# abhi1kumar/SUP-NeRF

Hardware: AMD Instinct MI355X
Metric: rays/sec at 4096 rays x 64 samples (fused render forward) (higher is better)
Workload: dtype f32

## Files before the change

sup-nerf_amd/csrc/snr_aux.hip:

```cpp
#include "snr_device.hpp"
#include "snr_host.hpp"

namespace snr {

__global__ void pack_fwd_kernel(const float* __restrict__ Wt, int n_out, int k_in, int n_chunks, float* __restrict__ dst) {
    const long long total = (long long)n_chunks * n_out * KC;
    for (long long i = blockIdx.x * (long long)blockDim.x + threadIdx.x; i < total; i += (long long)gridDim.x * blockDim.x) {
        const int kk = (int)(i % KC);
        const int row = (int)((i / KC) % n_out);
        const int c = (int)(i / ((long long)KC * n_out));
        const int k = c * KC + kk;
        dst[(long long)c * n_out * KC + chunk_pos(row, kk)] = (k < k_in) ? Wt[(long long)row * k_in + k] : 0.f;
    }
}

__global__ void pack_bwd_kernel(const float* __restrict__ Wt, int n_out, int k_in, int rows_pad, float* __restrict__ dst) {
    const int n_chunks = n_out / KC;
    const long long total = (long long)n_chunks * rows_pad * KC;
    for (long long i = blockIdx.x * (long long)blockDim.x + threadIdx.x; i < total; i += (long long)gridDim.x * blockDim.x) {
        const int kk = (int)(i % KC);
        const int row = (int)((i / KC) % rows_pad);
        const int c = (int)(i / ((long long)KC * rows_pad));
        const int n = c * KC + kk;
        dst[(long long)c * rows_pad * KC + chunk_pos(row, kk)] = (row < k_in) ? Wt[(long long)n * k_in + row] : 0.f;
    }
}

__global__ void copy_pad_kernel(const float* __restrict__ src, int n, float* __restrict__ dst, int n_pad) {
    const int i = blockIdx.x * blockDim.x + threadIdx.x;
    if (i < n_pad) dst[i] = (i < n) ? src[i] : 0.f;
}

__global__ void __launch_bounds__(256) composite_fwd_kernel(const float* __restrict__ sigmas, const float* __restrict__ rgbs,
                                                            const float* __restrict__ zv, int z_mode, int flags, long long n_rays,
                                                            long long rays_per_obj, int S, float* __restrict__ rgb,
                                                            float* __restrict__ depth, float* __restrict__ acc) {
    const int lane = threadIdx.x & 63;
    const long long wave0 = (blockIdx.x * (long long)blockDim.x + threadIdx.x) >> 6;
    const long long n_waves = ((long long)gridDim.x * blockDim.x) >> 6;
    const bool white = flags & SNR_WHITE_BKGD;
    for (long long ray = wave0; ray < n_rays; ray += n_waves) {
        const float* zrow = zv + (z_mode == SNR_Z_SHARED ? 0 : (z_mode == SNR_Z_PER_OBJECT ? (ray / rays_per_obj) * S : ray * S));
        const float* srow = sigmas + ray * S;
        const float* crow = rgbs + ray * S * 3;
        RayOut o = composite_ray_fwd(S, lane, white, [&](int k, float& sg, float& cr, float& cg, float& cb, float& z, float& zn) {
            sg = srow[k]; cr = crow[3 * k]; cg = crow[3 * k + 1]; cb = crow[3 * k + 2];
            z = zrow[k]; zn = (k < S - 1) ? zrow[k + 1] : 0.f;
        });
        if (lane == 0) {
            rgb[ray * 3] = o.r; rgb[ray * 3 + 1] = o.g; rgb[ray * 3 + 2] = o.b;
            depth[ray] = o.depth; acc[ray] = o.acc;
        }
    }
}

__global__ void __launch_bounds__(256) composite_fwd16_kernel(const float* __restrict__ sigmas, const float* __restrict__ rgbs,
                                                              const float* __restrict__ zv, int z_mode, int flags, long long n_rays,
                                                              long long rays_per_obj, int S, float* __restrict__ rgb,
                                                              float* __restrict__ depth, float* __restrict__ acc) {
    const int lane = threadIdx.x & 63, sub = lane & 15, grp = lane >> 4;
    const long long wave0 = (blockIdx.x * (long long)blockDim.x + threadIdx.x) >> 6;
    const long long n_waves = ((long long)gridDim.x * blockDim.x) >> 6;
    const bool white = flags & SNR_WHITE_BKGD;
    const int k0 = 4 * sub;
    const bool valid = k0 < S;
    for (long long base = wave0 * 4; base < n_rays; base += n_waves * 4) {
        const long long ray = base + grp;
        const bool live = ray < n_rays && valid;
        const long long rr = ray < n_rays ? ray : n_rays - 1;
        const float* zrow = zv + (z_mode == SNR_Z_SHARED ? 0 : (z_mode == SNR_Z_PER_OBJECT ? (rr / rays_per_obj) * S : rr * S));
        f32x4 sg = {0.f, 0.f, 0.f, 0.f}, z4 = sg, c0 = sg, c1 = sg, c2 = sg;
        if (live) {
            sg = *reinterpret_cast<const f32x4*>(sigmas + rr * S + k0);
            z4 = *reinterpret_cast<const f32x4*>(zrow + k0);
            const f32x4* cp = reinterpret_cast<const f32x4*>(rgbs + (rr * S + k0) * 3);
            c0 = cp[0]; c1 = cp[1]; c2 = cp[2];
        }
        const float zn = dpp_or<0x101>(0.f, z4[0]);
        const float zz[5] = {z4[0], z4[1], z4[2], z4[3], zn};
        const float cr[4] = {c0[0], c0[3], c1[2], c2[1]}, cg[4] = {c0[1], c1[0], c1[3], c2[2]}, cb[4] = {c0[2], c1[1], c2[0], c2[3]};
        float alpha[4], Al[4];
        float prod = 1.f;
#pragma unroll
        for (int e = 0; e < 4; ++e) {
            const int k = k0 + e;
            const float delta = (k == S - 1) ? LAST_DELTA : zz[e + 1] - zz[e];
            alpha[e] = 1.f - expf(-fmaxf(sg[e], 0.f) * delta);
            Al[e] = prod;
            prod *= live ? (1.f - alpha[e]) + TRANS_EPS : 1.f;
        }
        float incl = prod;
        incl *= dpp_or<0x111>(1.f, incl); incl *= dpp_or<0x112>(1.f, incl); incl *= dpp_or<0x114>(1.f, incl); incl *= dpp_or<0x118>(1.f, incl);
        const float excl = dpp_or<0x111>(1.f, incl);
        float sr = 0.f, sgc = 0.f, sb = 0.f, sd = 0.f, sw = 0.f, al = 0.f;
#pragma unroll
        for (int e = 0; e < 4; ++e) {
            const float A = excl * Al[e];
            const float w = live ? alpha[e] * A : 0.f;
            sr += w * cr[e]; sgc += w * cg[e]; sb += w * cb[e]; sd += w * zz[e]; sw += w;
            if (live && k0 + e == S - 1) al = A;
        }
        sr = row_sum(sr); sgc = row_sum(sgc); sb = row_sum(sb); sd = row_sum(sd); sw = row_sum(sw); al = row_sum(al);
        if (white) { const float bg = 1.f - sw; sr += bg; sgc += bg; sb += bg; }
        if (sub == 0 && ray < n_rays) {
            rgb[ray * 3] = sr; rgb[ray * 3 + 1] = sgc; rgb[ray * 3 + 2] = sb;
            depth[ray] = sd; acc[ray] = al;
        }
// ... 383 lines not shown
        v = (f < 3 + 3 * DIR_FREQ) ? sn : cs;
    }
    pe_dir[i] = v;
}

constexpr int RED_CHUNK = 32;
__global__ void __launch_bounds__(256) reduce_tiles_kernel(const float* __restrict__ in, long long tiles, int cols, float* __restrict__ out) {
    const long long n_chunks = (tiles + RED_CHUNK - 1) / RED_CHUNK;
    const long long chunk = blockIdx.x, obj = blockIdx.y;
    const long long t0 = chunk * RED_CHUNK;
    const long long t1 = (t0 + RED_CHUNK < tiles) ? t0 + RED_CHUNK : tiles;
    for (int c4 = threadIdx.x; c4 * 4 < cols; c4 += blockDim.x) {
        const float* p = in + (obj * tiles + t0) * cols + c4 * 4;
        f32x4 s0 = {0.f, 0.f, 0.f, 0.f}, s1 = s0;
        long long t = t0;
        for (; t + 1 < t1; t += 2) {
            s0 += *reinterpret_cast<const f32x4*>(p);
            s1 += *reinterpret_cast<const f32x4*>(p + cols);
            p += 2 * (long long)cols;
        }
        if (t < t1) s0 += *reinterpret_cast<const f32x4*>(p);
        *reinterpret_cast<f32x4*>(out + (obj * n_chunks + chunk) * cols + c4 * 4) = s0 + s1;
    }
}

}

using namespace snr;

int snr_bf16_pack_(const float* const* W, int sb, int tb, float* packed, void* stream_);

static thread_local const char* g_last_err = "";
int snr_check_launch_(void) {
    hipError_t e = hipGetLastError();
    if (e != hipSuccess) { g_last_err = hipGetErrorString(e); return SNR_E_LAUNCH; }
    return SNR_OK;
}

extern "C" {

int snr_abi_version(void) { return SNR_ABI_VERSION; }

const char* snr_last_hip_error(void) { return g_last_err; }

size_t snr_packed_bytes(int sb, int tb) {
    if (sb < 0 || tb < 0 || sb > MAX_BLOCKS || tb > MAX_BLOCKS) return 0;
    return (size_t)make_layout(sb, tb).total * sizeof(float);
}

size_t snr_mask_bytes(int64_t n_points, int sb, int tb) { return (size_t)mask_bytes(n_points, sb, tb); }

static inline int grid_for(long long total, int block = 256, int cap = 4096) {
    long long g = (total + block - 1) / block;
    return (int)(g < 1 ? 1 : (g > cap ? cap : g));
}

int snr_pack_weights(const float* const* t, int n_tensors, int sb, int tb, float* packed, void* stream_) {
    if (!t || !packed || sb < 0 || tb < 0 || sb > MAX_BLOCKS || tb > MAX_BLOCKS) return SNR_E_ARG;
    if (n_tensors != 2 * (sb + tb + 6)) return SNR_E_SHAPE;
    for (int i = 0; i < n_tensors; ++i) if (!t[i]) return SNR_E_ARG;
    hipStream_t st = (hipStream_t)stream_;
    const Layout L = make_layout(sb, tb);
    int ti = 0;
    auto Wp = [&](int i) { return t[2 * i]; };
    auto Bp = [&](int i) { return t[2 * i + 1]; };
    const int i_xyz = ti++;
    int i_shape[MAX_BLOCKS]; for (int j = 0; j < sb; ++j) i_shape[j] = ti++;
    const int i_encshape = ti++;
    const int i_sigma = ti++;
    const int i_view = ti++;
    int i_tex[MAX_BLOCKS]; for (int j = 0; j < tb; ++j) i_tex[j] = ti++;
    const int i_rgb0 = ti++;
    const int i_rgb2 = ti++;
    const long long c256 = 256 * KC;

    float* f = packed + L.fwd;
    auto fwd = [&](const float* Wsrc, int n_out, int k_in, int n_chunks) {
        pack_fwd_kernel<<<grid_for((long long)n_chunks * n_out * KC), 256, 0, st>>>(Wsrc, n_out, k_in, n_chunks, f);
        f += (long long)n_chunks * n_out * KC;
    };
    fwd(Wp(i_xyz), 256, D_XYZ, 2);
    for (int j = 0; j < sb; ++j) fwd(Wp(i_shape[j]), 256, 256, 8);
    fwd(Wp(i_encshape), 256, 256, 8);
    fwd(Wp(i_view), 256, 256 + D_DIR, 9);
    for (int j = 0; j < tb; ++j) fwd(Wp(i_tex[j]), 256, 256, 8);
    fwd(Wp(i_rgb0), 128, 256, 8);
    if (f - (packed + L.fwd) != L.fwd_floats) return SNR_E_SHAPE;

    float* b = packed + L.bwd;
    auto bwd = [&](const float* Wsrc, int n_out, int k_in, int rows_pad) {
        const int n_chunks = n_out / KC;
        pack_bwd_kernel<<<grid_for((long long)n_chunks * rows_pad * KC), 256, 0, st>>>(Wsrc, n_out, k_in, rows_pad, b);
        b += (long long)n_chunks * rows_pad * KC;
    };
    bwd(Wp(i_rgb0), 128, 256, 256);
    for (int j = tb - 1; j >= 0; --j) bwd(Wp(i_tex[j]), 256, 256, 256);
    bwd(Wp(i_view), 256, 256 + D_DIR, K_VIEW_PAD);
    bwd(Wp(i_encshape), 256, 256, 256);
    for (int j = sb - 1; j >= 0; --j) bwd(Wp(i_shape[j]), 256, 256, 256);
    bwd(Wp(i_xyz), 256, D_XYZ, K_XYZ_PAD);
    if (b - (packed + L.bwd) != L.bwd_floats) return SNR_E_SHAPE;
    (void)c256;

    auto vec = [&](const float* src, int n, long long off, int n_pad) {
        copy_pad_kernel<<<(n_pad + 255) / 256, 256, 0, st>>>(src, n, packed + off, n_pad);
    };
    vec(Bp(i_xyz), 256, L.bias + 256ll * layer_enc_xyz(), 256);
    for (int j = 0; j < sb; ++j) vec(Bp(i_shape[j]), 256, L.bias + 256ll * layer_shape(j), 256);
    vec(Bp(i_encshape), 256, L.bias + 256ll * layer_enc_shape(sb), 256);
    vec(Bp(i_view), 256, L.bias + 256ll * layer_viewdir(sb), 256);
    for (int j = 0; j < tb; ++j) vec(Bp(i_tex[j]), 256, L.bias + 256ll * layer_texture(sb, j), 256);
    vec(Bp(i_rgb0), 128, L.bias + 256ll * layer_rgb0(sb, tb), 256);
    vec(Wp(i_sigma), 256, L.sigma_w, 256);
    vec(Bp(i_sigma), 1, L.sigma_b, 4);
    vec(Wp(i_rgb2), 3 * 128, L.rgb2_w, 3 * 128);
    vec(Bp(i_rgb2), 3, L.rgb2_b, 4);
    {
        const float* Wl[MAX_BLOCKS * 2 + 4];
        int n = 0;
        Wl[n++] = Wp(i_xyz);
        for (int j = 0; j < sb; ++j) Wl[n++] = Wp(i_shape[j]);
        Wl[n++] = Wp(i_encshape);
        Wl[n++] = Wp(i_view);
        for (int j = 0; j < tb; ++j) Wl[n++] = Wp(i_tex[j]);
        Wl[n++] = Wp(i_rgb0);
        int rc = snr_bf16_pack_(Wl, sb, tb, packed, stream_);
        if (rc != SNR_OK) return rc;
    }
    return snr_check_launch_();
}

int snr_composite_fwd(const float* sigmas, const float* rgbs, const float* z_vals, int z_mode, int flags, int64_t n_rays,
                      int64_t rays_per_obj, int S, float* rgb, float* depth, float* acc, void* stream_) {
    if (n_rays == 0) return SNR_OK;
    if (!sigmas || !rgbs || !z_vals || !rgb || !depth || !acc) return SNR_E_ARG;
    if (n_rays < 0 || S < 1 || z_mode < 0 || z_mode > 2) return SNR_E_ARG;
    if (z_mode == SNR_Z_PER_OBJECT && (rays_per_obj < 1)) return SNR_E_SHAPE;
    if (rays_per_obj < 1) rays_per_obj = n_rays;
    const bool aligned = !(((uintptr_t)sigmas | (uintptr_t)rgbs | (uintptr_t)z_vals) & 15);
    if (S <= 64 && (S & 3) == 0 && aligned) {
        const int grid = grid_for(n_rays * 16, 256, 16384);
        composite_fwd16_kernel<<<grid, 256, 0, (hipStream_t)stream_>>>(sigmas, rgbs, z_vals, z_mode, flags, n_rays, rays_per_obj, S, rgb, depth, acc);
        return snr_check_launch_();
    }
    const int grid = grid_for(n_rays * 64, 256, 8192);
    composite_fwd_kernel<<<grid, 256, 0, (hipStream_t)stream_>>>(sigmas, rgbs, z_vals, z_mode, flags, n_rays, rays_per_obj, S, rgb, depth, acc);
    return snr_check_launch_();
}

int snr_scene_composite_fwd(const float* sigmas, const float* rgbs, const float* z_vals, int64_t n_pixels, int n_per_pixel, int run_length,
                            int flags, float* rgb, float* depth, float* acc, void* stream_) {
    if (n_pixels == 0) return SNR_OK;
    if (!sigmas || !rgbs || !z_vals || !rgb) return SNR_E_ARG;
    if (n_pixels < 0 || n_per_pixel < 1 || run_length < 0) return SNR_E_ARG;
    if (run_length > 0 && (n_per_pixel % run_length) != 0) return SNR_E_SHAPE;
    const size_t lds = (size_t)4 * 6 * n_per_pixel * sizeof(float);
    if (lds > 160 * 1024) return SNR_E_UNSUPPORTED;
    if (lds > 64 * 1024) {
        hipError_t e = hipFuncSetAttribute(reinterpret_cast<const void*>(scene_general_kernel<false>), hipFuncAttributeMaxDynamicSharedMemorySize, (int)lds);
        if (e != hipSuccess) return snr_check_launch_();
    }
    const int grid = grid_for(n_pixels * 64, 256, 8192);
    hipStream_t st = (hipStream_t)stream_;
    const bool fast = n_per_pixel <= 256 && (run_length == 32 || run_length == 64 || run_length == 128);
    if (fast) {
        if (run_length == 32) scene_fast_kernel<32><<<grid, 256, lds, st>>>(sigmas, rgbs, z_vals, n_pixels, n_per_pixel, flags, rgb, depth, acc);
        else if (run_length == 64) scene_fast_kernel<64><<<grid, 256, lds, st>>>(sigmas, rgbs, z_vals, n_pixels, n_per_pixel, flags, rgb, depth, acc);
        else scene_fast_kernel<128><<<grid, 256, lds, st>>>(sigmas, rgbs, z_vals, n_pixels, n_per_pixel, flags, rgb, depth, acc);
        scene_general_kernel<true><<<grid, 256, lds, st>>>(sigmas, rgbs, z_vals, n_pixels, n_per_pixel, run_length, flags, rgb, depth, acc);
    } else {
        scene_general_kernel<false><<<grid, 256, lds, st>>>(sigmas, rgbs, z_vals, n_pixels, n_per_pixel, run_length, flags, rgb, depth, acc);
    }
    return snr_check_launch_();
}

int snr_composite_bwd(const float* sigmas, const float* rgbs, const float* z_vals, int z_mode, int flags, int64_t n_rays,
                      int64_t rays_per_obj, int S, const float* d_rgb, const float* d_depth, const float* d_acc,
                      float* d_sigmas, float* d_rgbs, float* d_z, void* stream_) {
    if (n_rays == 0) return SNR_OK;
    if (!sigmas || !rgbs || !z_vals || !d_sigmas || !d_rgbs) return SNR_E_ARG;
    if (n_rays < 0 || S < 1 || z_mode < 0 || z_mode > 2) return SNR_E_ARG;
    if (d_z && z_mode != SNR_Z_PER_RAY) return SNR_E_UNSUPPORTED;
    if (S > 256) return SNR_E_UNSUPPORTED;
    if (rays_per_obj < 1) rays_per_obj = n_rays;
    const int grid = grid_for(n_rays * 64, 256, 8192);
    hipStream_t st = (hipStream_t)stream_;
#define SNR_LAUNCH_CB(N) composite_bwd_kernel<N><<<grid, 256, 0, st>>>(sigmas, rgbs, z_vals, z_mode, flags, n_rays, rays_per_obj, S, \
                                                                        d_rgb, d_depth, d_acc, d_sigmas, d_rgbs, d_z)
    if (S <= 64) SNR_LAUNCH_CB(1); else if (S <= 128) SNR_LAUNCH_CB(2); else if (S <= 192) SNR_LAUNCH_CB(3); else SNR_LAUNCH_CB(4);
#undef SNR_LAUNCH_CB
    return snr_check_launch_();
}

int snr_pe_points(const float* xyz, const float* viewdir, int64_t n_points, float* out, void* stream_) {
    if (n_points == 0) return SNR_OK;
    if (!xyz || !viewdir || !out || n_points < 0 || (((uintptr_t)out) & 15)) return SNR_E_ARG;
    pe_points_kernel<<<(unsigned)((n_points + 127) / 128), 256, 0, (hipStream_t)stream_>>>(xyz, viewdir, n_points, out);
    return snr_check_launch_();
}
// ... 63 lines not shown
```

sup-nerf_amd/csrc/snr_layout.h:

```cpp
#pragma once
#include <stdint.h>

#ifndef SNR_HD
#ifdef __HIPCC__
#define SNR_HD __host__ __device__
#else
#define SNR_HD
#endif
#endif

namespace snr {

constexpr int W = 256;
constexpr int W_RGB = 128;
constexpr int XYZ_FREQ = 10;
constexpr int DIR_FREQ = 4;
constexpr int D_XYZ = 3 + 6 * XYZ_FREQ;
constexpr int D_DIR = 3 + 6 * DIR_FREQ;
constexpr int KC = 32;
constexpr int K_XYZ_PAD = 64;
constexpr int K_VIEW_PAD = 288;
constexpr int MAX_BLOCKS = 8;

struct Layout {
    int sb, tb;
    int n_mfma_layers;
    int n_lat;
    int64_t fwd;
    int64_t bwd;
    int64_t bias;
    int64_t sigma_w;
    int64_t sigma_b;
    int64_t rgb2_w;
    int64_t rgb2_b;
    int64_t bf_fwd;
    int64_t bf_bwd;
    int64_t total;
    int64_t fwd_floats, bwd_floats;
    int64_t bf_fwd_bytes, bf_bwd_bytes;
};

constexpr int BF_CHUNK = 32768;
constexpr int BF_CHUNK_VIEW = 36864;

SNR_HD inline Layout make_layout(int sb, int tb) {
    Layout L;
    L.sb = sb; L.tb = tb;
    L.n_mfma_layers = sb + tb + 4;
    L.n_lat = sb + tb;
    const int64_t c256 = 256 * KC;
    L.fwd_floats = 2 * c256 + (int64_t)(sb + 1) * 8 * c256 + 9 * c256 + (int64_t)tb * 8 * c256 + 8 * (128 * KC);
    L.bwd_floats = 4 * c256 + (int64_t)tb * 8 * c256 + 8 * (288 * KC) + (int64_t)(sb + 1) * 8 * c256 + 8 * (64 * KC);
    int64_t o = 0;
    L.fwd = o; o += L.fwd_floats;
    L.bwd = o; o += L.bwd_floats;
    L.bias = o; o += (int64_t)L.n_mfma_layers * 256;
    L.sigma_w = o; o += 256;
    L.sigma_b = o; o += 4;
    L.rgb2_w = o; o += 3 * 128;
    L.rgb2_b = o; o += 4;
    L.bf_fwd_bytes = 2ll * BF_CHUNK + (int64_t)(sb + 1 + tb) * 8 * BF_CHUNK + 8ll * BF_CHUNK_VIEW + 4ll * BF_CHUNK;
    L.bf_bwd_bytes = 4ll * BF_CHUNK + (int64_t)tb * 8 * BF_CHUNK + 9ll * BF_CHUNK + (int64_t)(sb + 1) * 8 * BF_CHUNK + 2ll * BF_CHUNK;
    o = (o + 3) & ~3ll;
    L.bf_fwd = o; o += L.bf_fwd_bytes / 4;
    L.bf_bwd = o; o += L.bf_bwd_bytes / 4;
    L.total = o;
    return L;
}

SNR_HD inline int chunk_pos(int row, int kk) { return row * KC + ((((kk >> 2) ^ ((row >> 1) & 7)) << 2) | (kk & 3)); }

SNR_HD inline int layer_enc_xyz() { return 0; }
SNR_HD inline int layer_shape(int j ) { return 1 + j; }
SNR_HD inline int layer_enc_shape(int sb) { return 1 + sb; }
SNR_HD inline int layer_viewdir(int sb) { return 2 + sb; }
SNR_HD inline int layer_texture(int sb, int j) { return 3 + sb + j; }
SNR_HD inline int layer_rgb0(int sb, int tb) { return 3 + sb + tb; }

SNR_HD inline int n_relu_layers(int sb, int tb) { return sb + tb + 3; }
SNR_HD inline int64_t mask_bytes(int64_t n_points, int sb, int tb) {
    int64_t tiles = (n_points + 31) / 32;
    return tiles * n_relu_layers(sb, tb) * 64 * 16;
}

}
```

sup-nerf_amd/csrc/snr_mlp.hip:

```cpp
#include "snr_mlp_core.hpp"
#include "snr_host.hpp"

namespace snr {

#ifdef SNR_STAMPS
#define SNR32_STAMP(i) do { if (threadIdx.x == 0 && io.sigmas) { unsigned long long t_; asm volatile("s_memtime %0\n\ts_waitcnt lgkmcnt(0)" : "=s"(t_) :: "memory"); \
        reinterpret_cast<unsigned long long*>(io.sigmas)[(long long)blockIdx.x * 16 + 4 + (i)] = t_; } } while (0)
#else
#define SNR32_STAMP(i) do {} while (0)
#endif

__device__ __forceinline__ void decoder_forward_tile(const DecoderIO& io, const Layout& L, float* lds, long long gp , long long tile32,
                                                     float x, float y, float z, float dx, float dy, float dz,
                                                     float& o_sigma, float& o_r, float& o_g, float& o_b) {
    const int tid = threadIdx.x;
    const int lane = tid & 63, wave = tid >> 6;
    const int p = lane & 31, h = lane >> 5;
    const int sb = io.sb, tb = io.tb;
    const int n_relu = n_relu_layers(sb, tb);
    const bool tile_live = tile32 * 32 < io.n_points;
    const int dump_rows = (int)((io.n_points - tile32 * 32) < 32 ? (io.n_points - tile32 * 32) : 32);
    float* const dump_scr = lds + LDS_SCRATCH + wave * PE_WAVE;
    const float* bias = lds + LDS_BIAS;
    const float* heads = bias + L.n_mfma_layers * 256;
    const float* lat = io.latent + (gp / io.points_per_obj) * (long long)L.n_lat * 256;

    const long long wg_first = (long long)blockIdx.x * 128;
    const long long wg_last = wg_first + 127 < io.n_points ? wg_first + 127 : io.n_points - 1;
    const bool lat_in_lds = (wg_first / io.points_per_obj) == (wg_last / io.points_per_obj) && L.n_lat <= LDS_LAT_ROWS;
    const float* lat_wg = io.latent + (wg_first / io.points_per_obj) * (long long)L.n_lat * 256;
    float in[9][16];
    f32x16 acc[8];
    uint32_t mask[4];

    Pipe pipe;
    pipe_init(pipe, io.packed + L.fwd, lane);
    {
        chunk_dma(pipe.next, lds, 256, tid);
        pipe.next += 256 * KC;
        for (int r = wave; r < L.n_mfma_layers + 3; r += 4) {
            typedef const __attribute__((address_space(1))) void* gptr_t;
            typedef __attribute__((address_space(3))) void* lptr_t;
            __builtin_amdgcn_global_load_lds((gptr_t)(io.packed + L.bias + r * 256 + lane * 4), (lptr_t)(lds + LDS_BIAS + r * 256), 16, 0, 0);
        }
        if (lat_in_lds)
            for (int r = wave; r < L.n_lat; r += 4) {
                typedef const __attribute__((address_space(1))) void* gptr_t;
                typedef __attribute__((address_space(3))) void* lptr_t;
                __builtin_amdgcn_global_load_lds((gptr_t)(lat_wg + r * 256 + lane * 4), (lptr_t)(lds + LDS_LAT + r * 256), 16, 0, 0);
            }
        float* sc = lds + LDS_SCRATCH + wave * PE_WAVE + p * PE_ROW;
#pragma unroll 1
        for (int i = 0; i < 15; ++i) {
            const int q = 15 * h + i;
            float sn, cs;
            pe_sincos(ldexpf(pick3(x, y, z, q % 3), q / 3), &sn, &cs);
            sc[3 + q] = sn; sc[3 + 3 * XYZ_FREQ + q] = cs;
        }
#pragma unroll 1
        for (int i = 0; i < 6; ++i) {
            const int q = 6 * h + i;
            float sn, cs;
            pe_sincos(ldexpf(pick3(dx, dy, dz, q % 3), q / 3), &sn, &cs);
            sc[64 + 3 + q] = sn; sc[64 + 3 + 3 * DIR_FREQ + q] = cs;
        }
        if (h == 0) {
            sc[0] = x; sc[1] = y; sc[2] = z; sc[63] = 0.f;
            sc[64] = dx; sc[65] = dy; sc[66] = dz;
#pragma unroll
            for (int f = D_DIR; f < 32; ++f) sc[64 + f] = 0.f;
        }
        asm volatile("s_waitcnt vmcnt(0)" ::: "memory");
        __syncthreads();
#pragma unroll
        for (int c = 0; c < 2; ++c)
#pragma unroll
            for (int r = 0; r < 16; ++r) in[c][r] = sc[32 * c + 8 * (r >> 2) + 4 * h + (r & 3)];
#pragma unroll
        for (int r = 0; r < 16; ++r) in[8][r] = sc[64 + 8 * (r >> 2) + 4 * h + (r & 3)];
    }

    SNR32_STAMP(0);
    acc_init_bias<8, 8>(acc, bias, h);
    step<8, 8>(acc, in[0], pipe, lds, 256, tid);
    step<8, 8>(acc, in[1], pipe, lds, 256, tid);
    {
        const int la = latent_after(0, sb, tb);
        if (lat_in_lds && la >= 0) epilogue<8, 8, true>(acc, in, true, lds + LDS_LAT + la * 256, h, mask);
        else epilogue<8, 8, true>(acc, in, true, la >= 0 ? lat + la * 256 : nullptr, h, mask);
        if (tile_live) io.masks[(tile32 * n_relu + 0) * 64 + lane] = make_uint4(mask[0], mask[1], mask[2], mask[3]);
        if (io.act && tile_live) dump_operand_staged<8>(in, io.act + ((long long)0 * io.n_points + tile32 * 32) * 256, dump_rows, dump_scr, lane);
    }

    SNR32_STAMP(1);
    const int li_encshape = sb + 1, li_view = sb + 2, li_last = sb + tb + 2;
    o_sigma = 0.f;
#pragma unroll 1
    for (int li = 1; li <= li_last; ++li) {
        const bool is_view = (li == li_view);
        const int rows_after = (li == li_last) ? 128 : 256;
        acc_init_bias<8, 8>(acc, bias + li * 256, h);
        step<8, 8>(acc, in[0], pipe, lds, 256, tid);
        step<8, 8>(acc, in[1], pipe, lds, 256, tid);
        step<8, 8>(acc, in[2], pipe, lds, 256, tid);
        step<8, 8>(acc, in[3], pipe, lds, 256, tid);
        step<8, 8>(acc, in[4], pipe, lds, 256, tid);
        step<8, 8>(acc, in[5], pipe, lds, 256, tid);
        step<8, 8>(acc, in[6], pipe, lds, 256, tid);
        step<8, 8>(acc, in[7], pipe, lds, is_view ? 256 : rows_after, tid);
        if (is_view) step<8, 8>(acc, in[8], pipe, lds, rows_after, tid);
        const bool relu = (li != li_encshape);
        const int la = latent_after(li, sb, tb);
        if (lat_in_lds && la >= 0) epilogue<8, 8, true>(acc, in, relu, lds + LDS_LAT + la * 256, h, mask);
        else epilogue<8, 8, true>(acc, in, relu, la >= 0 ? lat + la * 256 : nullptr, h, mask);
        if (relu && tile_live)
            io.masks[(tile32 * n_relu + relu_slot(li, sb)) * 64 + lane] = make_uint4(mask[0], mask[1], mask[2], mask[3]);
        if (io.act && tile_live) dump_operand_staged<8>(in, io.act + ((long long)li * io.n_points + tile32 * 32) * 256, dump_rows, dump_scr, lane);
        if (li <= 6) SNR32_STAMP(1 + li);
        if (li == li_encshape) {
            const float* ws = heads;
            float part = 0.f;
#pragma unroll
            for (int t = 0; t < 8; ++t)
#pragma unroll
                for (int j = 0; j < 4; ++j) {
                    const f32x4 wv = *reinterpret_cast<const f32x4*>(ws + 32 * t + 8 * j + 4 * h);
#pragma unroll
                    for (int e = 0; e < 4; ++e) part = fmaf(wv[e], in[t][4 * j + e], part);
                }
            const float pre = sum_halves(part) + heads[L.sigma_b - L.sigma_w];
            o_sigma = pre > 20.f ? pre : log1pf(expf(pre));
        }
    }

    SNR32_STAMP(8);
    acc_init_bias<4, 8>(acc, bias + (li_last + 1) * 256, h);
    step<4, 8>(acc, in[0], pipe, lds, 128, tid);
    step<4, 8>(acc, in[1], pipe, lds, 128, tid);
    step<4, 8>(acc, in[2], pipe, lds, 128, tid);
    step<4, 8>(acc, in[3], pipe, lds, 128, tid);
    step<4, 8>(acc, in[4], pipe, lds, 128, tid);
    step<4, 8>(acc, in[5], pipe, lds, 128, tid);
    step<4, 8>(acc, in[6], pipe, lds, 128, tid);
    step<4, 8>(acc, in[7], pipe, lds, 0, tid);
    SNR32_STAMP(9);
    epilogue<4, 8, true>(acc, in, true, nullptr, h, mask);
    if (tile_live) io.masks[(tile32 * n_relu + (n_relu - 1)) * 64 + lane] = make_uint4(mask[0], mask[1], 0u, 0u);
    if (io.act && tile_live) dump_operand_staged<4>(in, io.act + ((long long)(li_last + 1) * io.n_points + tile32 * 32) * 256, dump_rows, dump_scr, lane);
    {
        const float* w2 = heads + (L.rgb2_w - L.sigma_w);
        float pr = 0.f, pg = 0.f, pb = 0.f;
#pragma unroll
        for (int t = 0; t < 4; ++t)
#pragma unroll
            for (int j = 0; j < 4; ++j) {
                const int n0 = 32 * t + 8 * j + 4 * h;
                const f32x4 wr = *reinterpret_cast<const f32x4*>(w2 + n0);
                const f32x4 wg = *reinterpret_cast<const f32x4*>(w2 + 128 + n0);
                const f32x4 wb = *reinterpret_cast<const f32x4*>(w2 + 256 + n0);
#pragma unroll
                for (int e = 0; e < 4; ++e) {
                    const float v = in[t][4 * j + e];
                    pr = fmaf(wr[e], v, pr); pg = fmaf(wg[e], v, pg); pb = fmaf(wb[e], v, pb);
                }
            }
        const float* b2 = heads + (L.rgb2_b - L.sigma_w);
        o_r = sum_halves(pr) + b2[0];
        o_g = sum_halves(pg) + b2[1];
        o_b = sum_halves(pb) + b2[2];
    }
}

__global__ void __launch_bounds__(256, 1)
decoder_train_fwd_kernel(DecoderIO io, Layout L, const float* __restrict__ xyz, const float* __restrict__ viewdir) {
    __shared__ __attribute__((aligned(16))) float lds[LDS_TOTAL];
    const int tid = threadIdx.x, lane = tid & 63, wave = tid >> 6, p = lane & 31;
    const long long tile128 = blockIdx.x;
    const long long gp_raw = tile128 * 128 + wave * 32 + p;
    const bool live = gp_raw < io.n_points;
    const long long gp = live ? gp_raw : io.n_points - 1;
    const float x = xyz[gp * 3], y = xyz[gp * 3 + 1], z = xyz[gp * 3 + 2];
    const float dx = viewdir[gp * 3], dy = viewdir[gp * 3 + 1], dz = viewdir[gp * 3 + 2];
    float sg, cr, cg, cb;
#ifdef SNR_STAMPS
    unsigned long long st_c0 = 0, st_r0 = 0;
    if (tid == 0) asm volatile("s_memtime %0\n\ts_memrealtime %1\n\ts_waitcnt lgkmcnt(0)" : "=s"(st_c0), "=s"(st_r0) :: "memory");
#endif
    decoder_forward_tile(io, L, lds, gp, tile128 * 4 + wave, x, y, z, dx, dy, dz, sg, cr, cg, cb);
#ifdef SNR_STAMPS
    if (tid == 0 && io.sigmas) {
        unsigned long long c1, r1;
        asm volatile("s_memtime %0\n\ts_memrealtime %1\n\ts_waitcnt lgkmcnt(0)" : "=s"(c1), "=s"(r1) :: "memory");
        unsigned long long* o = reinterpret_cast<unsigned long long*>(io.sigmas) + tile128 * 16;
        o[0] = st_c0; o[1] = st_r0; o[2] = c1; o[3] = r1;
    }
#else
    if (live && lane < 32) {
        if (io.sigmas) io.sigmas[gp] = sg;
        if (io.rgbs) { io.rgbs[gp * 3] = cr; io.rgbs[gp * 3 + 1] = cg; io.rgbs[gp * 3 + 2] = cb; }
    }
#endif
}

}

using namespace snr;

int snr_bf16_supported_(int sb, int tb, long long points_per_obj);
int snr_bf16_launch_fwd_(int mode, const DecoderIO& io, const Layout& L, const float* xyz, const float* viewdir, const RayGeom& g, float* rgb,
                         float* depth, float* acc, void* stream_);
int snr_fp32_fwd16_launch_(int mode, const DecoderIO& io, const Layout& L, const float* xyz, const float* viewdir, const RayGeom& g, float* rgb,
                           float* depth, float* acc, void* stream_);

extern "C" {
// ... 53 lines not shown
```

sup-nerf_amd/csrc/snr_mlp16.hip:

```cpp
#include "snr_mlp16_core.hpp"
#include "snr_host.hpp"

namespace snr {

struct Epi {
    float lo;
    const float* zlds;
    const float* zglb;
    float hi;
    float* dump;
};
struct EpiRegs { f32x4 z; };

__device__ __forceinline__ uint32_t spread_nibbles(uint32_t m16) {
    return ((m16 >> 12) & 0xFu) | (((m16 >> 8) & 0xFu) << 8) | (((m16 >> 4) & 0xFu) << 16) | ((m16 & 0xFu) << 24);
}

template <bool LATLDS>
__device__ __forceinline__ EpiRegs epi_load(const Epi& c, int T, int g) {
    EpiRegs e;
    e.z = f32x4{0.f, 0.f, 0.f, 0.f};
    if (LATLDS) e.z = *reinterpret_cast<const f32x4*>(c.zlds + 16 * T + 4 * g);
    else if (c.zglb) e.z = *reinterpret_cast<const f32x4*>(c.zglb + 16 * T + 4 * g);
    return e;
// ... 55 lines not shown
            for (int k = (gi * 4) / NG; k < ((gi + 1) * 4) / NG; ++k) epi_value<MASKS>(accP[2 * ch + 1], xb, c, e, 3 - k, m16);
            if (DUMP && gi == NG - 1) *reinterpret_cast<f32x4*>(c.dump + 16 * (2 * ch + 1)) = xb;
        });
        if (ch & 1) { mw[ch >> 1] = m16; m16 = 0u; }
        if (ch == 7) {
            tile_mma<NT, true>(accC, accP, xb, wb + ring.aoff[1], a0, a1, nullptr);
        } else {
            tile_mma<NT, false>(accC, accP, xb, wb + ring.aoff[1], a0, a1, nullptr, [&](int gi) {
                if (gi == 0) e = epi_load<LATLDS>(c, 2 * ch + 2, g);
#pragma unroll
                for (int k = (gi * 4) / NG; k < ((gi + 1) * 4) / NG; ++k) epi_value<MASKS>(accP[2 * ch + 2], xa, c, e, 3 - k, m16);
                if (DUMP && gi == NG - 1) *reinterpret_cast<f32x4*>(c.dump + 16 * (2 * ch + 2)) = xa;
            });
        }
        ring_turn(ring);
    }
}

__device__ __forceinline__ void store_masks16x4(uint4* __restrict__ dst , const uint32_t (&mw)[4], int wave, int lane) {
    const int n = lane & 15, g = lane >> 4;
    uint32_t w[4];
#pragma unroll
    for (int i = 0; i < 4; ++i) {
        const uint32_t mine = spread_nibbles(mw[i]) << (4 * (g >> 1));
        w[i] = mine | (uint32_t)__shfl_xor((int)mine, 32, 64);
    }
    if (g < 2) dst[16 * (wave & 1) + n + 32 * g] = make_uint4(w[0], w[1], w[2], w[3]);
}

#ifdef SNR_STAMPS
#define SNR16_STAMP(i) do { if (io.sigmas && lane == 0) { unsigned long long t_; asm volatile("s_memtime %0\n\ts_waitcnt lgkmcnt(0)" : "=s"(t_) :: "memory"); \
        reinterpret_cast<unsigned long long*>(io.sigmas)[(tile_wg * WAVES + wave) * 8 + (i)] = t_; } } while (0)
#define SNR16_STAMP_HWID(i) do { if (io.sigmas && lane == 0) { unsigned a_, b_; asm volatile("s_getreg_b32 %0, hwreg(HW_REG_HW_ID)\n\ts_getreg_b32 %1, hwreg(HW_REG_XCC_ID)" : "=s"(a_), "=s"(b_)); \
        reinterpret_cast<unsigned long long*>(io.sigmas)[(tile_wg * WAVES + wave) * 8 + (i)] = (unsigned long long)a_ | ((unsigned long long)b_ << 32); } } while (0)
#else
#define SNR16_STAMP(i) do {} while (0)
#define SNR16_STAMP_HWID(i) do {} while (0)
#endif

template <int MODE, int WAVES, bool LATLDS, bool MASKS, bool DUMP>
__global__ void __launch_bounds__(WAVES * 64, 2)
decoder_fwd16_kernel(DecoderIO io, Layout L, Lds16 lo, const float* __restrict__ xyz, const float* __restrict__ viewdir, RayGeom gm,
                     float* __restrict__ out_rgb, float* __restrict__ out_depth, float* __restrict__ out_acc) {
    extern __shared__ __attribute__((aligned(16))) float lds[];
    constexpr int WGP = WAVES * 16;
    const int tid = threadIdx.x, lane = tid & 63, wave = tid >> 6, n = lane & 15, g = lane >> 4;
    const long long tile_wg = blockIdx.x;
    const long long gp_raw = tile_wg * WGP + wave * 16 + n;
    const bool live = gp_raw < io.n_points;
    const long long gp = live ? gp_raw : io.n_points - 1;
    const long long tile32 = tile_wg * (WAVES / 2) + (wave >> 1);
    const bool tile_live = tile32 * 32 < io.n_points;
    const int sb = io.sb, tb = io.tb;
    const int n_relu = n_relu_layers(sb, tb);
    SNR16_STAMP(0);
    __builtin_amdgcn_s_setprio(3);
    float px, py, pz, dx, dy, dz, zc = 0.f;
    if (MODE == 0) {
        px = xyz[gp * 3]; py = xyz[gp * 3 + 1]; pz = xyz[gp * 3 + 2];
        dx = viewdir[gp * 3]; dy = viewdir[gp * 3 + 1]; dz = viewdir[gp * 3 + 2];
    } else {
        const PointId id = point_id(gm, tile_wg, WGP, wave * 16 + n, live);
        const SamplePoint sp = make_sample(gm, id.ray, id.s, id.obj);
        px = sp.x; py = sp.y; pz = sp.z; dx = sp.dx; dy = sp.dy; dz = sp.dz; zc = sp.zc;
    }
    const float* bias = lds + lo.bias;
    const float* heads = bias + L.n_mfma_layers * 256;
    const float* zero = lds + lo.zero;
    const float* lat_lane = io.latent + (gp / io.points_per_obj) * (long long)L.n_lat * 256;
    const float* lat_wg = io.latent + ((tile_wg * WGP) / io.points_per_obj) * (long long)L.n_lat * 256;

    Ring16 ring;
    ring.cur = 0;
    Dma16 dm;
    dm.voff = lane * 16u + 4096u;
    dm.lds0 = __builtin_amdgcn_readfirstlane((unsigned)(size_t)(__attribute__((address_space(3))) float*)lds);
    dm.wave = __builtin_amdgcn_readfirstlane(wave);
    {
        const int sw = (n >> 1) & 7;
        ring.aoff[0] = n * KC + (((0 + g) ^ sw) << 2);
        ring.aoff[1] = n * KC + (((4 + g) ^ sw) << 2);
    }
    constexpr long long C256 = 256 * KC;
    const int li_encshape = sb + 1, li_view = sb + 2, li_last = sb + tb + 2;
    const float* const stream = io.packed + L.fwd;
    auto layer_base = [&](int li) { return stream + 2 * C256 + (long long)(li - 1) * 8 * C256 + (li > li_view ? C256 : 0); };
    auto layer_first = [&](int li) { return layer_base(li) + (li == li_view ? 8 * C256 : 0); };
    f32x4 xin[4], xd[2];
    {
        chunk_dma16<WAVES>(dm, stream, lds, lds, 256);
        for (int r = dm.wave; r < L.n_mfma_layers + 3; r += WAVES) row_dma16(dm, io.packed + L.bias + r * 256, lds + lo.bias + r * 256, lds);
        if (LATLDS)
            for (int r = dm.wave; r < L.n_lat; r += WAVES) row_dma16(dm, lat_wg + r * 256, lds + lo.lat + r * 256, lds);
        if (tid < 64) *reinterpret_cast<f32x4*>(lds + lo.zero + 4 * tid) = f32x4{0.f, 0.f, 0.f, 0.f};
        float* sc = lds + lo.scratch + wave * PE_WAVE16 + n * PE_ROW;
#pragma unroll 1
        for (int i = 0; i < 8; i += 2) {
            const int q = 8 * g + i;
            if (q < 3 * XYZ_FREQ) {
                f32x2 sn, cs;
                pe_sincos2(f32x2{ldexpf(pick3(px, py, pz, q % 3), q / 3), ldexpf(pick3(px, py, pz, (q + 1) % 3), (q + 1) / 3)}, &sn, &cs);
                sc[3 + q] = sn[0]; sc[3 + 3 * XYZ_FREQ + q] = cs[0];
                sc[4 + q] = sn[1]; sc[4 + 3 * XYZ_FREQ + q] = cs[1];
            }
        }
        {
            const int q = 3 * g;
            f32x2 sn, cs;
            pe_sincos2(f32x2{ldexpf(pick3(dx, dy, dz, q % 3), q / 3), ldexpf(pick3(dx, dy, dz, (q + 1) % 3), (q + 1) / 3)}, &sn, &cs);
            sc[64 + 3 + q] = sn[0]; sc[64 + 3 + 3 * DIR_FREQ + q] = cs[0];
            sc[64 + 4 + q] = sn[1]; sc[64 + 4 + 3 * DIR_FREQ + q] = cs[1];
            float s1, c1;
            pe_sincos(ldexpf(pick3(dx, dy, dz, (q + 2) % 3), (q + 2) / 3), &s1, &c1);
            sc[64 + 5 + q] = s1; sc[64 + 5 + 3 * DIR_FREQ + q] = c1;
        }
        if (g == 0) {
            sc[0] = px; sc[1] = py; sc[2] = pz; sc[63] = 0.f;
            sc[64] = dx; sc[65] = dy; sc[66] = dz;
#pragma unroll
            for (int f = D_DIR; f < 32; ++f) sc[64 + f] = 0.f;
        }
        asm volatile("s_waitcnt vmcnt(0)" ::: "memory");
        __syncthreads();
#pragma unroll
        for (int T = 0; T < 4; ++T)
#pragma unroll
            for (int r = 0; r < 4; ++r) xin[T][r] = sc[16 * T + 4 * g + r];
#pragma unroll
        for (int T = 0; T < 2; ++T)
#pragma unroll
            for (int r = 0; r < 4; ++r) xd[T][r] = sc[64 + 16 * T + 4 * g + r];
        if (WAVES == 4) __syncthreads();
    }

    __builtin_amdgcn_s_setprio(0);
    SNR16_STAMP(1);
    f32x4 accP[16];
    {
        f32x4 accC[16];
        f32x4 a0, a1;
        acc_from_bias<16>(accC, bias, g);
#pragma unroll
        for (int ch = 0; ch < 2; ++ch) {
            chunk_dma16<WAVES>(dm, ch == 0 ? stream + C256 : layer_first(1), lds + (ring.cur ^ 1) * WBUF16, lds, 256);
            const float* wb = lds + ring.cur * WBUF16;
            first_pair(a0, a1, wb + ring.aoff[0]);
            tile_mma<16, false>(accC, accP, xin[2 * ch], wb + ring.aoff[0], a0, a1, wb + ring.aoff[1]);
            if (ch == 1) tile_mma<16, true>(accC, accP, xin[2 * ch + 1], wb + ring.aoff[1], a0, a1, nullptr);
            else tile_mma<16, false>(accC, accP, xin[2 * ch + 1], wb + ring.aoff[1], a0, a1, nullptr);
            ring_turn(ring);
        }
    }

    SNR16_STAMP(2);
    uint32_t mw[4] = {0u, 0u, 0u, 0u};
    float o_sigma = 0.f;
    float pos_inf = __builtin_inff();
    asm volatile("" : "+v"(pos_inf));
    float* const dump_lane = DUMP ? io.act + gp * 256 + 4 * g : nullptr;
    auto epi_of = [&](int lp) {
        const int la = latent_after(lp, sb, tb);
        Epi c;
        c.lo = (lp != li_encshape) ? 0.f : -__builtin_inff();
        c.zlds = (la >= 0) ? lds + lo.lat + la * 256 : zero;
        c.zglb = (la >= 0) ? lat_lane + la * 256 : nullptr;
        c.hi = pos_inf;
        c.dump = DUMP ? dump_lane + (long long)lp * io.n_points * 256 : nullptr;
        return c;
    };
    auto after_layer_input = [&](int lp) {
        if (MASKS && lp != li_encshape && tile_live) store_masks16x4(io.masks + (tile32 * n_relu + relu_slot(lp, sb)) * 64, mw, wave, lane);
    };
#pragma unroll 1
    for (int li = 1; li <= li_last; ++li) {
        const int lp = li - 1;
        const Epi c = epi_of(lp);
        if (li == li_view) {
            SNR16_STAMP(3);
            float s = 0.f;
#pragma unroll
            for (int T = 0; T < 16; ++T) {
                const f32x4 ws = *reinterpret_cast<const f32x4*>(heads + 16 * T + 4 * g);
#pragma unroll
                for (int r = 0; r < 4; ++r) s = fmaf(ws[r], accP[T][r], s);
            }
            s += __shfl_xor(s, 16, 64);
            s += __shfl_xor(s, 32, 64);
            const float pre = s + heads[L.sigma_b - L.sigma_w];
            o_sigma = pre > 20.f ? pre : log1pf(expf(pre));
        }
        layer_from_acc<16, WAVES, LATLDS, MASKS, DUMP>(accP, ring, lds, bias + li * 256, c, g, dm, layer_base(li), li == li_view, xd, layer_first(li + 1),
                                                       (li == li_last) ? 128 : 256, mw);
        after_layer_input(lp);
    }
    SNR16_STAMP(4);
    {
        const Epi c = epi_of(li_last);
        layer_from_acc<8, WAVES, LATLDS, MASKS, DUMP>(accP, ring, lds, bias + (li_last + 1) * 256, c, g, dm, layer_base(li_last + 1), false, xd, nullptr, 0, mw);
        after_layer_input(li_last);
    }

    SNR16_STAMP(5);
    __builtin_amdgcn_s_setprio(3);
    float o_r, o_g, o_b;
    {
        const float* w2 = heads + (L.rgb2_w - L.sigma_w);
        float pr = 0.f, pg = 0.f, pb = 0.f;
        uint32_t m16 = 0u, mr[4] = {0u, 0u, 0u, 0u};
        float* const dmp = DUMP ? dump_lane + (long long)(li_last + 1) * io.n_points * 256 : nullptr;
#pragma unroll
        for (int T = 0; T < 8; ++T) {
            const f32x4 wr = *reinterpret_cast<const f32x4*>(w2 + 16 * T + 4 * g);
            const f32x4 wg = *reinterpret_cast<const f32x4*>(w2 + 128 + 16 * T + 4 * g);
            const f32x4 wb = *reinterpret_cast<const f32x4*>(w2 + 256 + 16 * T + 4 * g);
            f32x4 xv;
#pragma unroll
            for (int r = 3; r >= 0; --r) {
                float v = accP[T][r];
                m16 = __builtin_amdgcn_alignbit(m16, __float_as_uint(0.f - v), 31);
                v = fmaxf(v, 0.f);
                xv[r] = v;
            }
#pragma unroll
            for (int r = 0; r < 4; ++r) { pr = fmaf(wr[r], xv[r], pr); pg = fmaf(wg[r], xv[r], pg); pb = fmaf(wb[r], xv[r], pb); }
            if (DUMP) *reinterpret_cast<f32x4*>(dmp + 16 * T) = xv;
            if ((T & 3) == 3) { mr[T >> 2] = m16; m16 = 0u; }
        }
        if (MASKS && tile_live) store_masks16x4(io.masks + (tile32 * n_relu + (n_relu - 1)) * 64, mr, wave, lane);
        pr += __shfl_xor(pr, 16, 64); pr += __shfl_xor(pr, 32, 64);
        pg += __shfl_xor(pg, 16, 64); pg += __shfl_xor(pg, 32, 64);
        pb += __shfl_xor(pb, 16, 64); pb += __shfl_xor(pb, 32, 64);
        const float* b2 = heads + (L.rgb2_b - L.sigma_w);
        o_r = pr + b2[0]; o_g = pg + b2[1]; o_b = pb + b2[2];
    }

    SNR16_STAMP_HWID(6);
#ifndef SNR_STAMPS
    if (live && g == 0 && io.sigmas) io.sigmas[gp] = o_sigma;
#endif
    if (live && g == 0) {
        if (io.rgbs) { io.rgbs[gp * 3] = o_r; io.rgbs[gp * 3 + 1] = o_g; io.rgbs[gp * 3 + 2] = o_b; }
    }
    if (MODE == 1) {
        float* comp = lds + lo.comp;
        if (g == 0) {
            float* c = comp + (wave * 16 + n) * COMP_STRIDE;
            c[0] = o_sigma; c[1] = o_r; c[2] = o_g; c[3] = o_b; c[4] = zc;
        }
        __syncthreads();
        const int S = gm.S;
        const int rays_here = WGP / S;
        const bool white = gm.flags & SNR_WHITE_BKGD;
        for (int r = wave; r < rays_here; r += WAVES) {
            const long long ray = tile_wg * rays_here + r;
            if (ray >= gm.n_rays) break;
            const float* c0 = comp + r * S * COMP_STRIDE;
            RayOut o = composite_ray_fwd(S, lane, white, [&](int k, float& s_, float& r_, float& g_, float& b_, float& z_, float& zn_) {
                const float* c = c0 + k * COMP_STRIDE;
                s_ = c[0]; r_ = c[1]; g_ = c[2]; b_ = c[3]; z_ = c[4];
                zn_ = (k < S - 1) ? c[COMP_STRIDE + 4] : 0.f;
            });
            if (lane == 0) {
                out_rgb[ray * 3] = o.r; out_rgb[ray * 3 + 1] = o.g; out_rgb[ray * 3 + 2] = o.b;
                out_depth[ray] = o.depth; out_acc[ray] = o.acc;
            }
        }
    }
    SNR16_STAMP(7);
}

}

using namespace snr;


template <int MODE, int WAVES, bool LATLDS, bool MASKS, bool DUMP>
static int launch16(const DecoderIO& io, const Layout& L, const Lds16& lo, const float* xyz, const float* viewdir, const RayGeom& g, float* rgb,
                    float* depth, float* acc, hipStream_t st) {
    auto kern = decoder_fwd16_kernel<MODE, WAVES, LATLDS, MASKS, DUMP>;
    static bool attr_set = false;
    if (!attr_set) {
// ... 34 lines not shown
```

Measured before the change: 2.472 million.

## Fold linear enc_shape layer into view layer and sigma head

Removes the un-activated enc_shape linear layer from the forward MLP chain by precomputing its product with the view-direction weights and the sigma head on the device at pack time. The bias is carried through a constant-one input column, and the sigma head gets a folded weight column and bias. This drops one 256x256 MFMA layer per sample. In exchange it adds double-precision reductions in the sigma head, disables activation dumping in the folded path, and changes relu-mask indexing, which risks affecting numerics and the backward consistency.

```diff
diff --git a/sup-nerf_amd/csrc/snr_aux.hip b/sup-nerf_amd/csrc/snr_aux.hip
--- a/sup-nerf_amd/csrc/snr_aux.hip
+++ b/sup-nerf_amd/csrc/snr_aux.hip
@@ -23,6 +23,36 @@
         const int c = (int)(i / ((long long)KC * rows_pad));
         const int n = c * KC + kk;
         dst[(long long)c * rows_pad * KC + chunk_pos(row, kk)] = (row < k_in) ? Wt[(long long)n * k_in + row] : 0.f;
+    }
+}
+
+__global__ void pack_fold_view_kernel(const float* __restrict__ Wv, const float* __restrict__ Ws, const float* __restrict__ bs, float* __restrict__ fwd) {
+    constexpr int KV = 256 + D_DIR;
+    const int i = blockIdx.x * blockDim.x + threadIdx.x;
+    if (i >= 256 * K_VIEW_PAD) return;
+    const int row = i / K_VIEW_PAD, k = i - row * K_VIEW_PAD;
+    float v = 0.f;
+    if (k < 256 || k == K_FOLD_ONE) {
+        double s = 0.0;
+        for (int j = 0; j < 256; ++j) s = fma((double)Wv[row * KV + j], (double)(k < 256 ? Ws[j * 256 + k] : bs[j]), s);
+        v = (float)s;
+    } else if (k < KV) {
+        v = Wv[row * KV + k];
+    }
+    fwd[(long long)(k / KC) * 256 * KC + chunk_pos(row, k % KC)] = v;
+}
+
+__global__ void pack_fold_head_kernel(const float* __restrict__ ws, const float* __restrict__ Ws, const float* __restrict__ bs,
+                                      const float* __restrict__ bsig, float* __restrict__ xyz_chunk1, float* __restrict__ fold_b) {
+    const int i = blockIdx.x * blockDim.x + threadIdx.x;
+    if (i < 256) {
+        double s = 0.0;
+        for (int j = 0; j < 256; ++j) s = fma((double)ws[j], (double)Ws[j * 256 + i], s);
+        xyz_chunk1[chunk_pos(i, KC - 1)] = (float)s;
+    } else if (i == 256) {
+        double s = (double)bsig[0];
+        for (int j = 0; j < 256; ++j) s = fma((double)ws[j], (double)bs[j], s);
+        fold_b[0] = (float)s;
     }
 }
 
@@ -572,7 +602,9 @@
     fwd(Wp(i_xyz), 256, D_XYZ, 2);
     for (int j = 0; j < sb; ++j) fwd(Wp(i_shape[j]), 256, 256, 8);
     fwd(Wp(i_encshape), 256, 256, 8);
-    fwd(Wp(i_view), 256, 256 + D_DIR, 9);
+    float* const fview = f;
+    f += 9 * c256;
+    pack_fold_view_kernel<<<256 * K_VIEW_PAD / 256, 256, 0, st>>>(Wp(i_view), Wp(i_encshape), Bp(i_encshape), fview);
     for (int j = 0; j < tb; ++j) fwd(Wp(i_tex[j]), 256, 256, 8);
     fwd(Wp(i_rgb0), 128, 256, 8);
     if (f - (packed + L.fwd) != L.fwd_floats) return SNR_E_SHAPE;
@@ -590,7 +622,6 @@
     for (int j = sb - 1; j >= 0; --j) bwd(Wp(i_shape[j]), 256, 256, 256);
     bwd(Wp(i_xyz), 256, D_XYZ, K_XYZ_PAD);
     if (b - (packed + L.bwd) != L.bwd_floats) return SNR_E_SHAPE;
-    (void)c256;
 
     auto vec = [&](const float* src, int n, long long off, int n_pad) {
         copy_pad_kernel<<<(n_pad + 255) / 256, 256, 0, st>>>(src, n, packed + off, n_pad);
@@ -605,6 +636,7 @@
     vec(Bp(i_sigma), 1, L.sigma_b, 4);
     vec(Wp(i_rgb2), 3 * 128, L.rgb2_w, 3 * 128);
     vec(Bp(i_rgb2), 3, L.rgb2_b, 4);
+    pack_fold_head_kernel<<<2, 256, 0, st>>>(Wp(i_sigma), Wp(i_encshape), Bp(i_encshape), Bp(i_sigma), packed + L.fwd + c256, packed + L.sigma_fold_b);
     {
         const float* Wl[MAX_BLOCKS * 2 + 4];
         int n = 0;
diff --git a/sup-nerf_amd/csrc/snr_layout.h b/sup-nerf_amd/csrc/snr_layout.h
--- a/sup-nerf_amd/csrc/snr_layout.h
+++ b/sup-nerf_amd/csrc/snr_layout.h
@@ -31,6 +31,7 @@
     int64_t bias;
     int64_t sigma_w;
     int64_t sigma_b;
+    int64_t sigma_fold_b;
     int64_t rgb2_w;
     int64_t rgb2_b;
     int64_t bf_fwd;
@@ -57,6 +58,7 @@
     L.bias = o; o += (int64_t)L.n_mfma_layers * 256;
     L.sigma_w = o; o += 256;
     L.sigma_b = o; o += 4;
+    L.sigma_fold_b = L.sigma_b + 1;
     L.rgb2_w = o; o += 3 * 128;
     L.rgb2_b = o; o += 4;
     L.bf_fwd_bytes = 2ll * BF_CHUNK + (int64_t)(sb + 1 + tb) * 8 * BF_CHUNK + 8ll * BF_CHUNK_VIEW + 4ll * BF_CHUNK;
@@ -67,6 +69,9 @@
     L.total = o;
     return L;
 }
+
+constexpr int K_FOLD_ONE = 256 + D_DIR;
+SNR_HD inline int fold_to_ref(int li, int sb) { return li <= sb ? li : li + 1; }
 
 SNR_HD inline int chunk_pos(int row, int kk) { return row * KC + ((((kk >> 2) ^ ((row >> 1) & 7)) << 2) | (kk & 3)); }
 
diff --git a/sup-nerf_amd/csrc/snr_mlp.hip b/sup-nerf_amd/csrc/snr_mlp.hip
--- a/sup-nerf_amd/csrc/snr_mlp.hip
+++ b/sup-nerf_amd/csrc/snr_mlp.hip
@@ -68,7 +68,7 @@
             sc[0] = x; sc[1] = y; sc[2] = z; sc[63] = 0.f;
             sc[64] = dx; sc[65] = dy; sc[66] = dz;
 #pragma unroll
-            for (int f = D_DIR; f < 32; ++f) sc[64 + f] = 0.f;
+            for (int f = D_DIR; f < 32; ++f) sc[64 + f] = (f == K_FOLD_ONE - 256) ? 1.f : 0.f;
         }
         asm volatile("s_waitcnt vmcnt(0)" ::: "memory");
         __syncthreads();
@@ -130,6 +130,19 @@
                 }
             const float pre = sum_halves(part) + heads[L.sigma_b - L.sigma_w];
             o_sigma = pre > 20.f ? pre : log1pf(expf(pre));
+            if (io.act && tile_live) {
+                asm volatile("s_waitcnt vmcnt(0)" ::: "memory");
+                const int pr = (lane & 31) < dump_rows ? (lane & 31) : dump_rows - 1;
+                const float* hrow = io.act + ((long long)(li - 1) * io.n_points + tile32 * 32 + pr) * 256 + 4 * h;
+#pragma unroll
+                for (int t = 0; t < 8; ++t)
+#pragma unroll
+                    for (int j = 0; j < 4; ++j) {
+                        const f32x4 v = *reinterpret_cast<const f32x4*>(hrow + 32 * t + 8 * j);
+#pragma unroll
+                        for (int e = 0; e < 4; ++e) in[t][4 * j + e] = v[e];
+                    }
+            }
         }
     }
 
diff --git a/sup-nerf_amd/csrc/snr_mlp16.hip b/sup-nerf_amd/csrc/snr_mlp16.hip
--- a/sup-nerf_amd/csrc/snr_mlp16.hip
+++ b/sup-nerf_amd/csrc/snr_mlp16.hip
@@ -161,10 +161,14 @@
         ring.aoff[1] = n * KC + (((4 + g) ^ sw) << 2);
     }
     constexpr long long C256 = 256 * KC;
-    const int li_encshape = sb + 1, li_view = sb + 2, li_last = sb + tb + 2;
+    const int li_view = sb + 1, li_last = li_view + tb;
     const float* const stream = io.packed + L.fwd;
-    auto layer_base = [&](int li) { return stream + 2 * C256 + (long long)(li - 1) * 8 * C256 + (li > li_view ? C256 : 0); };
+    auto layer_base = [&](int li) {
+        const int lr = fold_to_ref(li, sb);
+        return stream + 2 * C256 + (long long)(lr - 1) * 8 * C256 + (lr > sb + 2 ? C256 : 0);
+    };
     auto layer_first = [&](int li) { return layer_base(li) + (li == li_view ? 8 * C256 : 0); };
+    const float wfold = tid < 256 ? io.packed[L.fwd + C256 + chunk_pos(tid, KC - 1)] : 0.f;
     f32x4 xin[4], xd[2];
     {
         chunk_dma16<WAVES>(dm, stream, lds, lds, 256);
@@ -197,10 +201,11 @@
             sc[0] = px; sc[1] = py; sc[2] = pz; sc[63] = 0.f;
             sc[64] = dx; sc[65] = dy; sc[66] = dz;
 #pragma unroll
-            for (int f = D_DIR; f < 32; ++f) sc[64 + f] = 0.f;
+            for (int f = D_DIR; f < 32; ++f) sc[64 + f] = (f == K_FOLD_ONE - 256) ? 1.f : 0.f;
         }
         asm volatile("s_waitcnt vmcnt(0)" ::: "memory");
         __syncthreads();
+        if (tid < 256) lds[lo.bias + L.n_mfma_layers * 256 + tid] = wfold;
 #pragma unroll
         for (int T = 0; T < 4; ++T)
 #pragma unroll
@@ -236,11 +241,12 @@
     float o_sigma = 0.f;
     float pos_inf = __builtin_inff();
     asm volatile("" : "+v"(pos_inf));
-    float* const dump_lane = DUMP ? io.act + gp * 256 + 4 * g : nullptr;
+    static_assert(!DUMP, "the folded forward has no enc_shape activations to dump");
+    float* const dump_lane = nullptr;
     auto epi_of = [&](int lp) {
-        const int la = latent_after(lp, sb, tb);
+        const int la = latent_after(fold_to_ref(lp, sb), sb, tb);
         Epi c;
-        c.lo = (lp != li_encshape) ? 0.f : -__builtin_inff();
+        c.lo = 0.f;
         c.zlds = (la >= 0) ? lds + lo.lat + la * 256 : zero;
         c.zglb = (la >= 0) ? lat_lane + la * 256 : nullptr;
         c.hi = pos_inf;
@@ -248,7 +254,7 @@
         return c;
     };
     auto after_layer_input = [&](int lp) {
-        if (MASKS && lp != li_encshape && tile_live) store_masks16x4(io.masks + (tile32 * n_relu + relu_slot(lp, sb)) * 64, mw, wave, lane);
+        if (MASKS && tile_live) store_masks16x4(io.masks + (tile32 * n_relu + lp) * 64, mw, wave, lane);
     };
 #pragma unroll 1
     for (int li = 1; li <= li_last; ++li) {
@@ -256,26 +262,26 @@
         const Epi c = epi_of(lp);
         if (li == li_view) {
             SNR16_STAMP(3);
-            float s = 0.f;
+            double s = 0.0;
 #pragma unroll
             for (int T = 0; T < 16; ++T) {
                 const f32x4 ws = *reinterpret_cast<const f32x4*>(heads + 16 * T + 4 * g);
 #pragma unroll
-                for (int r = 0; r < 4; ++r) s = fmaf(ws[r], accP[T][r], s);
+                for (int r = 0; r < 4; ++r) s = fma((double)ws[r], (double)fmaxf(accP[T][r], 0.f), s);
             }
             s += __shfl_xor(s, 16, 64);
             s += __shfl_xor(s, 32, 64);
-            const float pre = s + heads[L.sigma_b - L.sigma_w];
+            const float pre = (float)(s + (double)heads[L.sigma_fold_b - L.sigma_w]);
             o_sigma = pre > 20.f ? pre : log1pf(expf(pre));
         }
-        layer_from_acc<16, WAVES, LATLDS, MASKS, DUMP>(accP, ring, lds, bias + li * 256, c, g, dm, layer_base(li), li == li_view, xd, layer_first(li + 1),
+        layer_from_acc<16, WAVES, LATLDS, MASKS, DUMP>(accP, ring, lds, bias + fold_to_ref(li, sb) * 256, c, g, dm, layer_base(li), li == li_view, xd, layer_first(li + 1),
                                                        (li == li_last) ? 128 : 256, mw);
         after_layer_input(lp);
     }
     SNR16_STAMP(4);
     {
         const Epi c = epi_of(li_last);
-        layer_from_acc<8, WAVES, LATLDS, MASKS, DUMP>(accP, ring, lds, bias + (li_last + 1) * 256, c, g, dm, layer_base(li_last + 1), false, xd, nullptr, 0, mw);
+        layer_from_acc<8, WAVES, LATLDS, MASKS, DUMP>(accP, ring, lds, bias + (li_last + 2) * 256, c, g, dm, layer_base(li_last + 1), false, xd, nullptr, 0, mw);
         after_layer_input(li_last);
     }
 
```

Measured after the change: 2.858 million, median of 6. 1.16x the previous value.
